# BurntSushi/aho-corasick

Measured on NVIDIA B200. Metric: haystack_scan_throughput, higher is better.
Workload: dtype u8

## Files before the change

### aho-corasick_b200/csrc/acb_api.cu

```cuda
#include <cuda_runtime.h>

#include <algorithm>
#include <chrono>
#include <cstdio>
#include <cstdlib>
#include <cstring>
#include <atomic>
#include <pthread.h>
#include <condition_variable>
#include <functional>
#include <mutex>
#include <thread>
#include <new>
#include <vector>

#include "../../include/acb200.h"
#include "../../include/acb200_debug.h"
#include "acb_build.hpp"
#include "acb_comm.hpp"
#include "acb_device.cuh"

using acb::DfaDev;
using acb::HostDfa;

namespace {

#define CK(expr)                                                                       \
  do {                                                                                 \
    cudaError_t e_ = (expr);                                                           \
    if (e_ != cudaSuccess) {                                                           \
      std::fprintf(stderr, "acb200: CUDA error %s at %s:%d: %s\n", cudaGetErrorName(e_), \
                   __FILE__, __LINE__, cudaGetErrorString(e_));                        \
      return ACG_E_CUDA;                                                               \
    }                                                                                  \
  } while (0)

struct Workspace {
  cudaStream_t stream = nullptr, copy_stream = nullptr;
  cudaEvent_t ev0 = nullptr, ev1 = nullptr, ev2 = nullptr, ev3 = nullptr;
  uint64_t cap = 0;
  uint64_t* d_keys[2] = {nullptr, nullptr};
  uint32_t* d_pids[2] = {nullptr, nullptr};
  unsigned long long* d_counter = nullptr;
  unsigned long long* h_counter = nullptr;
  void* d_temp = nullptr;
  size_t temp_bytes = 0;
  uint64_t* h_keys = nullptr;
  uint32_t* h_pids = nullptr;
  uint64_t h_cap = 0;
  uint8_t* d_hay = nullptr;
  uint64_t d_hay_cap = 0;
  uint64_t* d_scratch = nullptr;
  uint8_t* d_flags = nullptr;
  void* d_temp2 = nullptr;
  size_t temp2_bytes = 0;
  uint64_t chain_cap = 0;
  uint64_t* d_seq = nullptr;
  uint64_t seq_cap = 0;
  uint64_t* h_seq = nullptr;
  uint64_t h_seq_cap = 0;
  acg_stats stats{};
  uint8_t* h_stage[2] = {nullptr, nullptr};
  uint64_t h_stage_cap = 0;
  cudaEvent_t stage_ev[2] = {nullptr, nullptr};
};

}

struct PrefilterPlan {
  bool supported = false;
  uint32_t k = 0, kmask = 0, fold = 0, mult = 1, mult3 = 1, shift = 0, log_bits = 0;
  uint32_t stride = 1;
  uint32_t key_shift = 8;
  bool wide = false;
  bool brute = false;
  uint32_t dup_shift = 0;
  double fill = 0;
  uint64_t n_grams = 0;
  std::vector<uint32_t> bitmap;
  bool dense = false;
  std::vector<uint64_t> amap;
  uint32_t amap_log = 0;
  uint32_t bs_n = 0;
  uint8_t bs_byte[3] = {0, 0, 0};
  uint8_t bs_back[3] = {0, 0, 0};
};

struct acg_dfa {
  HostDfa h;
  std::vector<uint16_t> depth16;
  PrefilterPlan pf;
  uint32_t* d_bitmap = nullptr;
  uint2* d_amap = nullptr;
  bool has_empty = false;
  uint32_t max_list_len = 0;
  bool on_device = false;
  bool dev_touched = false;
  int device = -1;
  uint32_t* d_trans = nullptr;
  uint8_t* d_classes = nullptr;
  uint32_t* d_moff = nullptr;
  uint32_t* d_mpids = nullptr;
  uint32_t* d_plens = nullptr;
  uint16_t* d_depth16 = nullptr;
  DfaDev dev{};
  int engine_override = ACG_ENGINE_AUTO;
  uint64_t pipeline_chunk = 64ull << 20;
  mutable bool bytescan_inert = false;
  uint32_t experiment = 0;
  mutable std::mutex mu;
  static constexpr size_t kMaxWorkspaces = 4;
  mutable std::vector<Workspace*> ws_all, ws_free;
  mutable std::condition_variable ws_cv;
  mutable acg_stats last_stats{};
};

namespace {

thread_local Workspace* tls_ws = nullptr;
thread_local const acg_dfa* tls_stats_owner = nullptr;
thread_local acg_stats tls_stats{};
Workspace& cur_ws() { return *tls_ws; }

int init_workspace(Workspace& w) {
  CK(cudaStreamCreateWithFlags(&w.stream, cudaStreamNonBlocking));
  CK(cudaStreamCreateWithFlags(&w.copy_stream, cudaStreamNonBlocking));
  CK(cudaEventCreate(&w.ev0));
  CK(cudaEventCreate(&w.ev1));
  CK(cudaEventCreate(&w.ev2));
  CK(cudaEventCreate(&w.ev3));
  CK(cudaMalloc(&w.d_counter, 64));
  CK(cudaMallocHost(&w.h_counter, 64));
  return ACG_OK;
}

void destroy_workspace(Workspace& w) {
  if (w.stream) cudaStreamSynchronize(w.stream);
  for (int i = 0; i < 2; ++i) { cudaFree(w.d_keys[i]); cudaFree(w.d_pids[i]); }
  cudaFree(w.d_counter); cudaFree(w.d_temp); cudaFree(w.d_hay); cudaFree(w.d_seq);
  cudaFree(w.d_scratch); cudaFree(w.d_flags); cudaFree(w.d_temp2);
  if (w.h_counter) cudaFreeHost(w.h_counter);
  if (w.h_keys) cudaFreeHost(w.h_keys);
  if (w.h_pids) cudaFreeHost(w.h_pids);
  if (w.h_seq) cudaFreeHost(w.h_seq);
  for (int i = 0; i < 2; ++i) {
    if (w.h_stage[i]) cudaFreeHost(w.h_stage[i]);
    if (w.stage_ev[i]) cudaEventDestroy(w.stage_ev[i]);
  }
  if (w.ev0) cudaEventDestroy(w.ev0);
  if (w.ev1) cudaEventDestroy(w.ev1);
  if (w.ev2) cudaEventDestroy(w.ev2);
  if (w.ev3) cudaEventDestroy(w.ev3);
  if (w.stream) cudaStreamDestroy(w.stream);
  if (w.copy_stream) cudaStreamDestroy(w.copy_stream);
}

struct WsLease {
  const acg_dfa* a;
  Workspace* w = nullptr;
  Workspace* prev;
  int rc = ACG_OK;
  explicit WsLease(const acg_dfa* a_) : a(a_), prev(tls_ws) {
    std::unique_lock<std::mutex> lk(a->mu);
    for (;;) {
      if (!a->ws_free.empty()) { w = a->ws_free.back(); a->ws_free.pop_back(); break; }
      if (a->ws_all.size() < acg_dfa::kMaxWorkspaces) {
        w = new (std::nothrow) Workspace();
        if (!w) { rc = ACG_E_NOMEM; return; }
        a->ws_all.push_back(w);
        lk.unlock();
        int prev_dev = -1;
        cudaGetDevice(&prev_dev);
        if (prev_dev != a->device) cudaSetDevice(a->device);
        rc = init_workspace(*w);
        if (prev_dev != a->device && prev_dev >= 0) cudaSetDevice(prev_dev);
        break;
      }
      a->ws_cv.wait(lk);
    }
    if (rc == ACG_OK) { w->stats = acg_stats{}; tls_ws = w; }
  }
  Workspace* detach() {
    Workspace* out = w;
    if (w) { tls_stats = w->stats; tls_stats_owner = a; tls_ws = prev; }
    w = nullptr;
    return out;
  }
  ~WsLease() {
    if (!w) return;
    tls_stats = w->stats;
    tls_stats_owner = a;
    tls_ws = prev;
    std::lock_guard<std::mutex> lk(a->mu);
    a->last_stats = w->stats;
    if (rc == ACG_OK) a->ws_free.push_back(w);
    a->ws_cv.notify_one();
  }
};

void release_workspace(const acg_dfa* a, Workspace* w) {
  if (!w) return;
  std::lock_guard<std::mutex> lk(a->mu);
  a->last_stats = w->stats;
  a->ws_free.push_back(w);
  a->ws_cv.notify_one();
}

int bits_for(uint64_t v) {
  int b = 0;
  while (v) { ++b; v >>= 1; }
  return b;
}

uint32_t bloom_hash2(uint32_t x) {
  x ^= x >> 16;
  x *= 0x7feb352du;
  x ^= x >> 15;
  x *= 0x846ca68bu;
  x ^= x >> 16;
  return x;
}

// ... 412 lines not shown
}

int ensure_tuple_cap(Workspace& w, uint64_t cap) {
  if (cap <= w.cap) return ACG_OK;
  for (int i = 0; i < 2; ++i) {
    if (w.d_keys[i]) cudaFree(w.d_keys[i]);
    if (w.d_pids[i]) cudaFree(w.d_pids[i]);
    w.d_keys[i] = nullptr;
    w.d_pids[i] = nullptr;
  }
  if (w.d_temp) { cudaFree(w.d_temp); w.d_temp = nullptr; }
  w.cap = 0;
  for (int i = 0; i < 2; ++i) {
    CK(cudaMalloc(&w.d_keys[i], cap * 8));
    CK(cudaMalloc(&w.d_pids[i], cap * 4));
  }
  size_t tb = 0;
  CK(acb::sort_pairs(nullptr, tb, w.d_keys[0], w.d_keys[1], w.d_pids[0], w.d_pids[1], cap, 64, w.stream));
  CK(cudaMalloc(&w.d_temp, std::max<size_t>(tb, 16)));
  w.temp_bytes = tb;
  w.cap = cap;
  return ACG_OK;
}

int ensure_host_staging(Workspace& w, uint64_t n) {
  if (n <= w.h_cap) return ACG_OK;
  if (w.h_keys) cudaFreeHost(w.h_keys);
  if (w.h_pids) cudaFreeHost(w.h_pids);
  w.h_keys = nullptr;
  w.h_pids = nullptr;
  w.h_cap = 0;
  const uint64_t cap = std::max<uint64_t>(n, 1 << 16);
  CK(cudaMallocHost(&w.h_keys, cap * 8));
  CK(cudaMallocHost(&w.h_pids, cap * 4));
  w.h_cap = cap;
  return ACG_OK;
}

int ensure_hay(Workspace& w, uint64_t bytes) {
  if (bytes <= w.d_hay_cap) return ACG_OK;
  if (w.d_hay) cudaFree(w.d_hay);
  w.d_hay = nullptr;
  w.d_hay_cap = 0;
  const uint64_t cap = ((bytes + (1ull << 20)) >> 20) << 20;
  CK(cudaMalloc(&w.d_hay, cap));
  w.d_hay_cap = cap;
  return ACG_OK;
}

int ensure_seq(Workspace& w, uint64_t cap) {
  if (cap > w.seq_cap) {
    if (w.d_seq) cudaFree(w.d_seq);
    w.d_seq = nullptr;
    w.seq_cap = 0;
    CK(cudaMalloc(&w.d_seq, cap * 24));
    w.seq_cap = cap;
  }
  if (cap > w.h_seq_cap) {
    if (w.h_seq) cudaFreeHost(w.h_seq);
    w.h_seq = nullptr;
    w.h_seq_cap = 0;
    CK(cudaMallocHost(&w.h_seq, cap * 24));
    w.h_seq_cap = cap;
  }
  return ACG_OK;
}

int check_anchored(int have, int want_anchored) {
  if (have == ACG_START_BOTH) return ACG_OK;
  if (have == ACG_START_UNANCHORED) return want_anchored ? ACG_E_INVALID_INPUT_ANCHORED : ACG_OK;
  return want_anchored ? ACG_OK : ACG_E_INVALID_INPUT_UNANCHORED;
}
bool span_ok(uint64_t hay_len, uint64_t s, uint64_t e) { return e <= hay_len && s <= e + 1; }
int check_start(const HostDfa& h, int anchored) {
  if (anchored) return h.start_anchored_id == 0 ? ACG_E_INVALID_INPUT_ANCHORED : ACG_OK;
  return h.start_unanchored_id == 0 ? ACG_E_INVALID_INPUT_UNANCHORED : ACG_OK;
}

struct TupleResult {
  uint64_t n = 0;
  int sorted_buf = 0;
};

int run_walk_overlapping(const acg_dfa* a, const uint8_t* d_hay, uint64_t readable, uint64_t span_start,
                         uint64_t span_end, TupleResult* res) {
  Workspace& w = cur_ws();
  const uint64_t n_bytes = span_end - span_start;
  if (a->max_list_len >= (1u << acb::kTieBits)) return ACG_E_INVALID_ARG;
  if (n_bytes >= (1ull << (64 - acb::kTieBits))) return ACG_E_INVALID_ARG;
  int dev_sms = 148;
  cudaDeviceGetAttribute(&dev_sms, cudaDevAttrMultiProcessorCount, a->device);
  const uint64_t target_lanes = uint64_t(dev_sms) * 2048;
  uint64_t seg_len = (n_bytes + target_lanes - 1) / std::max<uint64_t>(target_lanes, 1);
  seg_len = std::max<uint64_t>(seg_len, 256);
  seg_len = (seg_len + 15) & ~15ull;
  const uint64_t n_segs = std::max<uint64_t>((n_bytes + seg_len - 1) / seg_len, 1);
  uint64_t cap = std::max<uint64_t>(w.cap, std::max<uint64_t>(1 << 20, n_bytes / 256));
  for (int attempt = 0; attempt < 8; ++attempt) {
    int rc = ensure_tuple_cap(w, cap);
    if (rc) return rc;
    CK(cudaMemsetAsync(w.d_counter, 0, 8, w.stream));
    acb::WalkLaunch p;
    p.hay = d_hay;
    p.hay_len = readable;
    p.span_start = span_start;
    p.span_end = span_end;
    p.seg_len = seg_len;
    p.n_segs = n_segs;
    p.keys = w.d_keys[0];
    p.pids = w.d_pids[0];
    p.counter = w.d_counter;
    p.cap = w.cap;
    CK(cudaEventRecord(w.ev0, w.stream));
    CK(acb::launch_walk_overlapping(a->dev, p, w.stream));
    CK(cudaEventRecord(w.ev1, w.stream));
    CK(cudaMemcpyAsync(w.h_counter, w.d_counter, 8, cudaMemcpyDeviceToHost, w.stream));
    CK(cudaStreamSynchronize(w.stream));
    cur_ws().stats.launches += 1;
    const uint64_t want = *w.h_counter;
    if (want > w.cap) { cap = want + want / 8 + 1024; continue; }
    res->n = want;
    cur_ws().stats.raw_matches = want;
    float ms = 0;
    cudaEventElapsedTime(&ms, w.ev0, w.ev1);
    cur_ws().stats.scan_ms = ms;
    if (want > 1) {
      size_t tb = w.temp_bytes;
      const int end_bit = std::min(64, acb::kTieBits + bits_for(n_bytes + 1));
      CK(cudaEventRecord(w.ev2, w.stream));
      CK(acb::sort_pairs(w.d_temp, tb, w.d_keys[0], w.d_keys[1], w.d_pids[0], w.d_pids[1], want, end_bit,
                         w.stream));
      CK(cudaEventRecord(w.ev3, w.stream));
      CK(cudaStreamSynchronize(w.stream));
      cudaEventElapsedTime(&ms, w.ev2, w.ev3);
      cur_ws().stats.order_ms = ms;
      cur_ws().stats.launches += 8;
      res->sorted_buf = 1;
    } else {
      res->sorted_buf = 0;
    }
    return ACG_OK;
  }
  return ACG_E_NOMEM;
}

int enqueue_prefilter_range(const acg_dfa* a, const uint8_t* d_hay, uint64_t readable,
                            uint64_t span_start, uint64_t span_end, uint64_t scan_lo,
                            uint64_t scan_hi, int mode, int dev_sms) {
  Workspace& w = cur_ws();
  const PrefilterPlan& pf = a->pf;
  const uintptr_t base = reinterpret_cast<uintptr_t>(d_hay);
  uint64_t lo = scan_lo + ((16 - ((base + scan_lo) & 15)) & 15);
  const uint64_t limit = std::min<uint64_t>(scan_hi, readable >= 20 ? readable - 20 : 0);
  uint64_t hi = lo;
  if (limit > lo) hi = lo + ((limit - lo) & ~15ull);
  if (lo > scan_hi) { lo = scan_hi; hi = scan_hi; }
  acb::PrefilterLaunch p;
  p.hay = d_hay;
  p.hay_len = readable;
  p.span_start = span_start;
  p.span_end = span_end;
  p.bitmap = a->d_bitmap;
  p.log_bits = pf.log_bits;
  p.k = pf.k;
  p.stride = pf.stride;
  p.geom = pf.wide ? 1 : 0;
  p.pair = 0;
  p.dyn = (a->experiment & ACG_EXP_STATIC_TILES) ? 0 : ((a->experiment & ACG_EXP_GLOBAL_TILES) ? 2 : 1);
  p.kmask = pf.kmask;
  p.fold = pf.fold;
  p.mult = pf.mult;
  p.mult3 = pf.mult3;
  p.key_shift = pf.key_shift;
  p.shift = pf.shift;
  p.dense = pf.dense ? 1 : 0;
  p.brute = pf.brute ? 1 : 0;
  p.mode = mode == 1 ? 1 : 0;
  p.first_only = mode == 2 ? 1 : 0;
  p.dup_shift = pf.dup_shift;
  p.scan_lo = scan_lo;
  p.scan_hi = scan_hi;
  p.region_lo = lo;
  p.region_hi = hi;
  p.keys = w.d_keys[0];
  p.pids = w.d_pids[0];
  p.counter = w.d_counter;
  p.cap = w.cap;
  p.bs_n = 0;
  for (int i = 0; i < 3; ++i) { p.bs_needle[i] = 0; p.bs_back[i] = 0; }
  if (pf.bs_n && !a->bytescan_inert && !(a->experiment & ACG_EXP_NO_BYTESCAN)) {
    p.bs_n = pf.bs_n;
    for (uint32_t i = 0; i < pf.bs_n; ++i) { p.bs_needle[i] = uint32_t(pf.bs_byte[i]) * 0x01010101u; p.bs_back[i] = pf.bs_back[i]; }
    CK(acb::launch_bytescan(a->dev, p, dev_sms, w.stream));
  } else {
    if (p.dyn == 2) CK(cudaMemsetAsync(w.d_counter + 2, 0, 8, w.stream));
    CK(acb::launch_prefilter(a->dev, p, dev_sms, w.stream));
  }
  cur_ws().stats.launches += 1;
  return ACG_OK;
}

int order_tuples(const acg_dfa* a, uint64_t want, uint64_t n_bytes, TupleResult* res) {
  Workspace& w = cur_ws();
  res->n = want;
  cur_ws().stats.raw_matches = want;
  if (want > 1) {
    size_t tb = w.temp_bytes;
    const int end_bit = std::min(64, acb::kTieBits + bits_for(n_bytes + 1));
    float ms = 0;
    CK(cudaEventRecord(w.ev2, w.stream));
    CK(acb::sort_pairs(w.d_temp, tb, w.d_keys[0], w.d_keys[1], w.d_pids[0], w.d_pids[1], want, end_bit,
                       w.stream));
    CK(cudaEventRecord(w.ev3, w.stream));
    CK(cudaStreamSynchronize(w.stream));
    cudaEventElapsedTime(&ms, w.ev2, w.ev3);
    cur_ws().stats.order_ms = ms;
    cur_ws().stats.launches += 8;
    res->sorted_buf = 1;
  } else {
    res->sorted_buf = 0;
  }
  return ACG_OK;
}

class CopyPool {
 public:
  static CopyPool& get() {
    static std::once_flag once;
    std::call_once(once, [] { pthread_atfork(nullptr, nullptr, [] { instance().store(nullptr); }); });
    CopyPool* p = instance().load(std::memory_order_acquire);
    if (!p) {
      CopyPool* fresh = new CopyPool;
      if (instance().compare_exchange_strong(p, fresh)) p = fresh;
    }
    return *p;
  }
  void copy(uint8_t* dst, const uint8_t* src, size_t n) {
    if (n < (4u << 20) || workers_.empty()) { std::memcpy(dst, src, n); return; }
    std::unique_lock<std::mutex> lk(mu_);
    busy_cv_.wait(lk, [&] { return !active_; });
    active_ = true;
    dst_ = dst; src_ = src; n_ = n;
    next_.store(0);
    pending_ = int(workers_.size());
    ++epoch_;
    cv_.notify_all();
    done_cv_.wait(lk, [&] { return pending_ == 0; });
    active_ = false;
    busy_cv_.notify_one();
  }

 private:
  static std::atomic<CopyPool*>& instance() {
    static std::atomic<CopyPool*> p{nullptr};
    return p;
  }
  CopyPool() {
    unsigned n = std::thread::hardware_concurrency();
    n = n >= 16 ? 8 : (n >= 4 ? n / 2 : 0);
    for (unsigned i = 0; i < n; ++i) workers_.emplace_back([this] { run(); });
    for (auto& t : workers_) t.detach();
  }
  void run() {
    uint64_t seen = 0;
    for (;;) {
      std::unique_lock<std::mutex> lk(mu_);
      cv_.wait(lk, [&] { return epoch_ != seen; });
      seen = epoch_;
      uint8_t* dst = dst_;
      const uint8_t* src = src_;
      const size_t n = n_;
      lk.unlock();
      constexpr size_t kSlice = 1u << 20;
      for (;;) {
        const size_t off = next_.fetch_add(kSlice);
        if (off >= n) break;
        std::memcpy(dst + off, src + off, std::min(kSlice, n - off));
      }
      lk.lock();
      if (--pending_ == 0) done_cv_.notify_one();
    }
  }
  std::mutex mu_;
  std::condition_variable cv_, done_cv_, busy_cv_;
  std::vector<std::thread> workers_;
  uint8_t* dst_ = nullptr;
  const uint8_t* src_ = nullptr;
  size_t n_ = 0;
  std::atomic<size_t> next_{0};
  int pending_ = 0;
  uint64_t epoch_ = 0;
  bool active_ = false;
};

bool is_pageable_host(const void* p) {
  cudaPointerAttributes attr;
  if (cudaPointerGetAttributes(&attr, p) != cudaSuccess) { cudaGetLastError(); return false; }
  return attr.type == cudaMemoryTypeUnregistered;
}

int ensure_stage(Workspace& w, uint64_t bytes) {
  if (bytes <= w.h_stage_cap) return ACG_OK;
  for (int i = 0; i < 2; ++i) {
    if (w.h_stage[i]) { cudaFreeHost(w.h_stage[i]); w.h_stage[i] = nullptr; }
    CK(cudaMallocHost(&w.h_stage[i], bytes));
    if (!w.stage_ev[i]) CK(cudaEventCreateWithFlags(&w.stage_ev[i], cudaEventDisableTiming));
  }
  w.h_stage_cap = bytes;
  return ACG_OK;
}

int run_prefilter(const acg_dfa* a, const uint8_t* d_hay, uint64_t readable, uint64_t span_start,
                  uint64_t span_end, int mode, TupleResult* res, const uint8_t* h_hay = nullptr,
                  uint64_t scan_lo = UINT64_MAX, uint64_t scan_hi = UINT64_MAX) {
  if (scan_lo == UINT64_MAX) { scan_lo = span_start; scan_hi = span_end; }
  Workspace& w = cur_ws();
  const uint64_t n_bytes = span_end - span_start;
  if (n_bytes >= (1ull << (64 - acb::kTieBits))) return ACG_E_INVALID_ARG;
  int dev_sms = 148;
  cudaDeviceGetAttribute(&dev_sms, cudaDevAttrMultiProcessorCount, a->device);
  uint64_t cap = std::max<uint64_t>(w.cap, std::max<uint64_t>(1 << 20, (scan_hi - scan_lo) / 256));
  bool copied = h_hay == nullptr;
  for (int attempt = 0; attempt < 8; ++attempt) {
    int rc = ensure_tuple_cap(w, cap);
    if (rc) return rc;
    CK(cudaMemsetAsync(w.d_counter, 0, 16, w.stream));
    CK(cudaEventRecord(w.ev0, w.stream));
    if (copied) {
      if ((rc = enqueue_prefilter_range(a, d_hay, readable, span_start, span_end, scan_lo, scan_hi, mode,
                                        dev_sms)))
        return rc;
    } else {
      const uint64_t chunk = a->pipeline_chunk;
      const uint64_t tail = std::min<uint64_t>(a->h.max_pattern_len, 1u << 30) + 64;
      uint64_t scanned = span_start;
      const bool staged = span_end - span_start >= std::min<uint64_t>(8u << 20, chunk) && is_pageable_host(h_hay + span_start);
      if (staged && (rc = ensure_stage(w, std::min<uint64_t>(chunk, span_end - span_start)))) return rc;
      bool stage_used[2] = {false, false};
      int stage_i = 0;
      CK(cudaEventRecord(w.ev2, w.copy_stream));
      for (uint64_t c0 = span_start; c0 < span_end; c0 += chunk) {
        const uint64_t c1 = std::min(span_end, c0 + chunk);
        const uint8_t* src = h_hay + c0;
        if (staged) {
          if (stage_used[stage_i]) CK(cudaEventSynchronize(w.stage_ev[stage_i]));
          CopyPool::get().copy(w.h_stage[stage_i], h_hay + c0, size_t(c1 - c0));
          src = w.h_stage[stage_i];
        }
        CK(cudaMemcpyAsync(const_cast<uint8_t*>(d_hay) + c0, src, c1 - c0, cudaMemcpyHostToDevice,
                           w.copy_stream));
        if (staged) {
          CK(cudaEventRecord(w.stage_ev[stage_i], w.copy_stream));
          stage_used[stage_i] = true;
          stage_i ^= 1;
        }
        CK(cudaEventRecord(w.ev3, w.copy_stream));
        CK(cudaStreamWaitEvent(w.stream, w.ev3, 0));
        const uint64_t upto = c1 == span_end ? span_end : (c1 > scanned + tail ? c1 - tail : scanned);
        if (upto > scanned || c1 == span_end) {
          if ((rc = enqueue_prefilter_range(a, d_hay, c1 == span_end ? readable : c1, span_start, span_end,
                                            scanned, upto, mode, dev_sms)))
            return rc;
          scanned = upto;
        }
      }
      copied = true;
    }
    CK(cudaEventRecord(w.ev1, w.stream));
    CK(cudaMemcpyAsync(w.h_counter, w.d_counter, 16, cudaMemcpyDeviceToHost, w.stream));
    CK(cudaStreamSynchronize(w.stream));
    const uint64_t want = w.h_counter[0];
    cur_ws().stats.candidates = w.h_counter[1];
    if (a->pf.bs_n && !a->bytescan_inert && scan_hi - scan_lo >= (1u << 16) && w.h_counter[1] > (scan_hi - scan_lo) / 64)
      a->bytescan_inert = true;
    float ms = 0;
    cudaEventElapsedTime(&ms, w.ev0, w.ev1);
    cur_ws().stats.scan_ms = ms;
    if (want > w.cap) { cap = want + want / 8 + 1024; continue; }
    return order_tuples(a, want, n_bytes, res);
  }
  return ACG_E_NOMEM;
}

int ensure_chain(Workspace& w, uint64_t n) {
  if (n <= w.chain_cap) return ACG_OK;
  if (w.d_scratch) cudaFree(w.d_scratch);
  if (w.d_flags) cudaFree(w.d_flags);
  if (w.d_temp2) cudaFree(w.d_temp2);
  w.d_scratch = nullptr; w.d_flags = nullptr; w.d_temp2 = nullptr; w.chain_cap = 0;
  const uint64_t cap = std::max<uint64_t>(n, 1 << 16);
  CK(cudaMalloc(&w.d_scratch, cap * 8));
  CK(cudaMalloc(&w.d_flags, cap));
  size_t t1 = 0, t2 = 0;
  CK(acb::scan_max_u64(nullptr, t1, w.d_scratch, cap, w.stream));
  CK(acb::select_flagged(nullptr, t2, w.d_keys[0], w.d_pids[0], w.d_flags, w.d_keys[1], w.d_pids[1],
                         w.d_counter, cap, w.stream));
  w.temp2_bytes = std::max(t1, t2);
  CK(cudaMalloc(&w.d_temp2, std::max<size_t>(w.temp2_bytes, 16)));
  w.chain_cap = cap;
  return ACG_OK;
}

int run_chain(const acg_dfa* a, int mode, TupleResult* r) {
  Workspace& w = cur_ws();
  if (r->n == 0) return ACG_OK;
  int rc = ensure_chain(w, r->n);
  if (rc) return rc;
  const int src = r->sorted_buf, dst = 1 - src;
  acb::ChainLaunch c;
  c.keys = w.d_keys[src];
  c.pids = w.d_pids[src];
  c.pattern_lens = a->d_plens;
  c.n = r->n;
  c.mode = mode;
  c.scratch_end = w.d_scratch;
  c.flags = w.d_flags;
  CK(cudaEventRecord(w.ev2, w.stream));
  CK(cudaMemsetAsync(w.d_flags, 0, r->n, w.stream));
  CK(acb::launch_chain_ends(c, w.stream));
  size_t tb = w.temp2_bytes;
  CK(acb::scan_max_u64(w.d_temp2, tb, w.d_scratch, r->n, w.stream));
  CK(acb::launch_chain_select(c, w.stream));
  tb = w.temp2_bytes;
  CK(acb::select_flagged(w.d_temp2, tb, w.d_keys[src], w.d_pids[src], w.d_flags, w.d_keys[dst],
                         w.d_pids[dst], w.d_counter, r->n, w.stream));
  CK(cudaEventRecord(w.ev3, w.stream));
  CK(cudaMemcpyAsync(w.h_counter, w.d_counter, 8, cudaMemcpyDeviceToHost, w.stream));
  CK(cudaStreamSynchronize(w.stream));
  float ms = 0;
  cudaEventElapsedTime(&ms, w.ev2, w.ev3);
  cur_ws().stats.order_ms += ms;
  cur_ws().stats.launches += 8;
  r->n = *w.h_counter;
  r->sorted_buf = dst;
  return ACG_OK;
}

int drain_tuples(const acg_dfa* a, const TupleResult& r, uint64_t span_start, acg_match* out,
                 uint64_t cap, uint64_t* n_out, uint64_t* fnv, int key_mode = 0) {
  Workspace& w = cur_ws();
  *n_out = r.n;
  if (fnv) *fnv = 0xcbf29ce484222325ull;
  if (r.n == 0) return ACG_OK;
  if (!fnv && r.n > cap) return ACG_E_OVERFLOW;
  int rc = ensure_host_staging(w, r.n);
  if (rc) return rc;
  CK(cudaEventRecord(w.ev0, w.stream));
  CK(cudaMemcpyAsync(w.h_keys, w.d_keys[r.sorted_buf], r.n * 8, cudaMemcpyDeviceToHost, w.stream));
  CK(cudaMemcpyAsync(w.h_pids, w.d_pids[r.sorted_buf], r.n * 4, cudaMemcpyDeviceToHost, w.stream));
  CK(cudaEventRecord(w.ev1, w.stream));
  CK(cudaStreamSynchronize(w.stream));
  float ms = 0;
  cudaEventElapsedTime(&ms, w.ev0, w.ev1);
  cur_ws().stats.d2h_ms += ms;
  const uint32_t* plens = a->h.pattern_lens.data();
  uint64_t hsh = 0xcbf29ce484222325ull;
  auto mix = [&](uint64_t v) {
    for (int k = 0; k < 8; ++k) { hsh ^= (v >> (8 * k)) & 0xFF; hsh *= 0x100000001b3ull; }
  };
  for (uint64_t i = 0; i < r.n; ++i) {
    const uint32_t pid = w.h_pids[i];
    uint64_t start, end;
// ... 541 lines not shown
  if (cudaMemcpy(t.data(), a->d_trans, t.size() * 4, cudaMemcpyDeviceToHost) != cudaSuccess) {
    cudaGetLastError();
    return ACG_E_CUDA;
  }
  h.trans.swap(t);
  return ACG_OK;
}

}

int acg_dfa_table(const acg_dfa* a, acg_dfa_desc* o) {
  if (!a || !o) return ACG_E_INVALID_ARG;
  if (int rc = fetch_table(a)) return rc;
  const HostDfa& h = a->h;
  o->trans = h.trans.data();
  o->trans_len = h.trans.size();
  o->stride2 = h.stride2;
  o->alphabet_len = h.alphabet_len;
  std::memcpy(o->byte_classes, h.classes, 256);
  o->max_special_id = h.max_special_id;
  o->max_match_id = h.max_match_id;
  o->start_unanchored_id = h.start_unanchored_id;
  o->start_anchored_id = h.start_anchored_id;
  o->match_offsets = h.match_offsets.data();
  o->match_pids = h.match_pids.data();
  o->pattern_lens = h.pattern_lens.data();
  o->n_patterns = uint32_t(h.pattern_lens.size());
  o->match_kind = uint32_t(h.match_kind);
  o->start_kind = uint32_t(h.start_kind);
  o->prefilter_kind = uint32_t(h.prefilter_kind);
  o->min_pattern_len = h.min_pattern_len;
  o->max_pattern_len = h.max_pattern_len;
  return ACG_OK;
}

uint64_t acg_dfa_state_len(const acg_dfa* a) { return a ? a->h.state_len : 0; }
int acg_kind(const acg_dfa* a) { return a ? a->h.reported_kind : 0; }
int acg_match_kind(const acg_dfa* a) { return a ? a->h.match_kind : 0; }
int acg_start_kind(const acg_dfa* a) { return a ? a->h.start_kind : 0; }
uint64_t acg_patterns_len(const acg_dfa* a) { return a ? a->h.pattern_lens.size() : 0; }
uint64_t acg_min_pattern_len(const acg_dfa* a) { return a ? a->h.min_pattern_len : 0; }
uint64_t acg_max_pattern_len(const acg_dfa* a) { return a ? a->h.max_pattern_len : 0; }
uint64_t acg_memory_usage(const acg_dfa* a) {
  if (!a) return 0;
  const HostDfa& h = a->h;
  return h.trans_len * 4 + (h.match_offsets.size() - 1) * 24 + h.match_pids.size() * 4 +
         h.pattern_lens.size() * 4;
}
int acg_prefilter_kind(const acg_dfa* a) { return a ? a->h.prefilter_kind : 0; }
int acg_packed_variant(const acg_dfa* a, int* fat, int* mask_len) {
  if (!a || !a->h.packed.active) return 0;
  if (fat) *fat = a->h.packed.fat;
  if (mask_len) *mask_len = a->h.packed.mask_len;
  return 1;
}

int acg_debug_prefilter_plan(const acg_dfa* a, acg_prefilter_plan* out) {
  if (!a || !out) return ACG_E_INVALID_ARG;
  const PrefilterPlan& pf = a->pf;
  *out = acg_prefilter_plan{};
  out->supported = pf.supported ? 1 : 0;
  out->brute = pf.brute ? 1 : 0;
  out->dense = pf.dense ? 1 : 0;
  out->stride = int32_t(pf.stride);
  out->wide = pf.wide ? 1 : 0;
  out->k = pf.k; out->kmask = pf.kmask; out->fold = pf.fold;
  out->mult = pf.mult; out->mult3 = pf.mult3; out->key_shift = pf.key_shift; out->shift = pf.shift; out->log_bits = pf.log_bits;
  out->bitmap = pf.bitmap.data(); out->bitmap_words = pf.bitmap.size();
  out->amap = pf.amap.data(); out->amap_log = pf.amap_log;
  out->depth16 = a->depth16.data(); out->n_rows = a->depth16.size();
  out->dup_shift = pf.dup_shift;
  out->bs_n = (pf.bs_n && !a->bytescan_inert) ? pf.bs_n : 0;
  for (int i = 0; i < 3; ++i) { out->bs_byte[i] = pf.bs_byte[i]; out->bs_back[i] = pf.bs_back[i]; }
  return ACG_OK;
}

int acg_debug_set_pipeline_chunk(acg_dfa* a, uint64_t bytes) {
  if (!a || bytes < 4096 || (bytes & 4095)) return ACG_E_INVALID_ARG;
  a->pipeline_chunk = bytes;
  return ACG_OK;
}

int acg_debug_set_experiment(acg_dfa* a, uint32_t flags) {
  if (!a || (flags & ~uint32_t(ACG_EXP_KEY24 | ACG_EXP_STATIC_TILES | ACG_EXP_NO_BYTESCAN | ACG_EXP_GLOBAL_TILES))) return ACG_E_INVALID_ARG;
  std::lock_guard<std::mutex> lock(a->mu);
  const uint32_t changed = a->experiment ^ flags;
  a->experiment = flags;
  if (changed & ACG_EXP_KEY24) {
    const size_t old_words = a->pf.bitmap.size();
    derive_metadata(a);
    if (a->on_device && a->d_bitmap && a->pf.supported) {
      if (a->pf.bitmap.size() != old_words) return ACG_E_INVALID_ARG;
      DeviceGuard guard(a->device);
      if (cudaMemcpy(a->d_bitmap, a->pf.bitmap.data(), old_words * 4, cudaMemcpyHostToDevice) != cudaSuccess) {
        cudaGetLastError();
        return ACG_E_CUDA;
      }
    }
  }
  return ACG_OK;
}

int acg_set_engine(acg_dfa* a, int engine) {
  if (!a || engine < ACG_ENGINE_AUTO || engine > ACG_ENGINE_SEQUENTIAL) return ACG_E_INVALID_ARG;
  a->engine_override = engine;
  return ACG_OK;
}
static acg_stats stats_for(const acg_dfa* a) {
  if (tls_stats_owner == a) return tls_stats;
  std::lock_guard<std::mutex> lk(a->mu);
  return a->last_stats;
}
int acg_last_engine(const acg_dfa* a) { return a ? stats_for(a).engine : 0; }
int acg_last_stats(const acg_dfa* a, acg_stats* out) {
  if (!a || !out) return ACG_E_INVALID_ARG;
  *out = stats_for(a);
  return ACG_OK;
}

int acg_find_overlapping(const acg_dfa* a, const uint8_t* hay, uint64_t hay_len, uint64_t span_start,
                         uint64_t span_end, int anchored, acg_match* out, uint64_t cap,
                         uint64_t* n_out) {
  return overlapping_impl(a, hay, false, hay_len, span_start, span_end, anchored, out, cap, n_out,
                          nullptr, nullptr);
}
int acg_find_overlapping_dev(const acg_dfa* a, const void* d_hay, uint64_t hay_len,
                             uint64_t span_start, uint64_t span_end, acg_match* out, uint64_t cap,
                             uint64_t* n_out, float* kernel_ms) {
  return overlapping_impl(a, static_cast<const uint8_t*>(d_hay), true, hay_len, span_start, span_end,
                          0, out, cap, n_out, nullptr, kernel_ms);
}
int acg_find_overlapping_devout(const acg_dfa* a, const void* d_hay, uint64_t hay_len,
                                uint64_t span_start, uint64_t span_end, uint64_t min_end,
                                uint64_t offset_add, void* d_out, uint64_t cap, uint64_t* n_out,
                                float* kernel_ms) {
  if (!d_out && cap) return ACG_E_INVALID_ARG;
  DevOut dv;
  dv.d_out = d_out;
  dv.min_end = min_end;
  dv.offset_add = offset_add;
  return overlapping_impl(a, static_cast<const uint8_t*>(d_hay), true, hay_len, span_start, span_end, 0,
                          nullptr, cap, n_out, nullptr, kernel_ms, &dv);
}
int acg_count_overlapping_dev(const acg_dfa* a, const void* d_hay, uint64_t hay_len,
                              uint64_t span_start, uint64_t span_end, uint64_t* n_out, uint64_t* fnv,
                              float* kernel_ms) {
  uint64_t dummy_fnv = 0;
  return overlapping_impl(a, static_cast<const uint8_t*>(d_hay), true, hay_len, span_start, span_end,
                          0, nullptr, 0, n_out, fnv ? fnv : &dummy_fnv, kernel_ms);
}

int acg_find_iter(const acg_dfa* a, const uint8_t* hay, uint64_t hay_len, uint64_t span_start,
                  uint64_t span_end, int anchored, acg_match* out, uint64_t cap, uint64_t* n_out) {
  return find_iter_impl(a, hay, false, hay_len, span_start, span_end, anchored, out, cap, n_out,
                        nullptr);
}
int acg_find_iter_dev(const acg_dfa* a, const void* d_hay, uint64_t hay_len, uint64_t span_start,
                      uint64_t span_end, acg_match* out, uint64_t cap, uint64_t* n_out,
                      float* kernel_ms) {
  return find_iter_impl(a, static_cast<const uint8_t*>(d_hay), true, hay_len, span_start, span_end, 0,
                        out, cap, n_out, kernel_ms);
}

int acg_find(const acg_dfa* a, const uint8_t* hay, uint64_t hay_len, uint64_t span_start,
             uint64_t span_end, int anchored, int earliest, acg_match* out, int* found) {
  if (!out || !found) return ACG_E_INVALID_ARG;
  *found = 0;
// ... 349 lines not shown
```

### aho-corasick_b200/csrc/acb_device.cuh

```cuda
#pragma once
#include <cuda_runtime.h>
#include <stdint.h>

namespace acb {

constexpr int kTieBits = 24;
constexpr uint64_t kTieMask = (1ull << kTieBits) - 1;
constexpr uint64_t kInvalidKey = ~0ull;

struct DfaDev {
  const uint32_t* trans;
  const uint8_t* classes;
  const uint32_t* match_offsets;
  const uint32_t* match_pids;
  const uint32_t* pattern_lens;
  const uint16_t* depth16;
  uint32_t stride2;
  uint32_t max_match_id;
  uint32_t start_unanchored_id;
  uint32_t start_anchored_id;
  uint32_t max_pattern_len;
  uint32_t min_pattern_len;
  const uint2* amap;
  uint32_t amap_shift;
// ... 28 lines not shown
  uint32_t n;
};
cudaError_t launch_dfa_fill_level(const FillLaunch& f, cudaStream_t s);

struct SeqLaunch {
  const uint8_t* hay;
  uint64_t span_start, span_end;
  int anchored;
  int match_kind;
  int earliest;
  int single;
  uint64_t* out;
  unsigned long long* counter;
  uint64_t cap;
};
cudaError_t launch_seq_find(const DfaDev& dfa, const SeqLaunch& p, cudaStream_t s);

struct PrefilterLaunch {
  const uint8_t* hay;
  uint64_t hay_len;
  uint64_t span_start, span_end;
  const uint32_t* bitmap;
  uint32_t log_bits;
  uint32_t k;
  uint32_t stride;
  uint16_t geom;
  uint16_t pair;
  uint32_t kmask;
  uint32_t fold;
  uint32_t mult;
  uint32_t mult3;
  uint32_t shift;
  int dense;
  int brute;
  int mode;
  int first_only;
  uint32_t dup_shift;
  uint64_t scan_lo, scan_hi;
  uint64_t region_lo, region_hi;
  uint64_t* keys;
  uint32_t* pids;
  unsigned long long* counter;
  uint64_t cap;
  uint32_t dyn;
  uint32_t bs_n;
  uint32_t bs_needle[3];
  uint32_t bs_back[3];
  uint32_t key_shift;
};
cudaError_t launch_prefilter(const DfaDev& dfa, const PrefilterLaunch& p, int sm_count, cudaStream_t s);
cudaError_t launch_bytescan(const DfaDev& dfa, const PrefilterLaunch& p, int sm_count, cudaStream_t s);

struct ChainLaunch {
  const uint64_t* keys;
  const uint32_t* pids;
  const uint32_t* pattern_lens;
  uint64_t n;
  int mode;
  uint64_t* scratch_end;
  uint8_t* flags;
};
cudaError_t launch_chain_ends(const ChainLaunch& c, cudaStream_t s);
cudaError_t launch_chain_select(const ChainLaunch& c, cudaStream_t s);
cudaError_t scan_max_u64(void* d_temp, size_t& temp_bytes, uint64_t* data, uint64_t n, cudaStream_t s);
cudaError_t select_flagged(void* d_temp, size_t& temp_bytes, const uint64_t* keys_in, const uint32_t* pids_in,
                           const uint8_t* flags, uint64_t* keys_out, uint32_t* pids_out,
                           unsigned long long* d_num_out, uint64_t n, cudaStream_t s);

struct ExpandLaunch {
  const uint64_t* keys;
  const uint32_t* pids;
  const uint32_t* pattern_lens;
  uint64_t n;
  uint64_t first;
  uint64_t span_start;
  uint64_t offset_add;
  uint64_t* out;
  int small = 0;
};
cudaError_t launch_expand(const ExpandLaunch& e, cudaStream_t s);
cudaError_t launch_lower_bound(const uint64_t* keys, uint64_t n, uint64_t bound_key,
                               unsigned long long* d_result, cudaStream_t s);

cudaError_t sort_pairs(void* d_temp, size_t& temp_bytes, const uint64_t* keys_in, uint64_t* keys_out,
                       const uint32_t* vals_in, uint32_t* vals_out, uint64_t n, int end_bit,
                       cudaStream_t s);

}
```

### aho-corasick_b200/csrc/acb_kernels.cu

```cuda
#include "acb_device.cuh"
#ifndef ACB_PTX_HEADER
#define ACB_PTX_HEADER "acb_ptx.cuh"
#endif
#include ACB_PTX_HEADER

#include <algorithm>
#include <cstdio>
#include <cstdlib>

#include <cub/device/device_radix_sort.cuh>

namespace acb {

namespace {

__device__ __noinline__ void emit_state_matches(const uint32_t* match_offsets, const uint32_t* match_pids,
                                                uint32_t row, uint64_t end_rel, uint64_t* keys, uint32_t* pids,
                                                unsigned long long* counter, uint64_t cap) {
  const uint32_t lo = match_offsets[row], hi = match_offsets[row + 1];
  const int lane = threadIdx.x & 31;
  for (uint32_t i = lo; i < hi; ++i) {
    const unsigned m = __activemask();
    const int leader = __ffs(m) - 1;
    unsigned long long base = 0;
// ... 120 lines not shown
    sid = d.trans[sid + d.classes[hay[at]]];
    if (sid <= d.max_match_id) {
      if (sid == 0) break;
      SeqMatch m = seq_get_match(d, sid, 0, at + 1);
      if (!(anchored && m.start > start)) {
        mat = m;
        have = true;
        if (earliest) break;
      }
    }
    ++at;
  }
  if (have) *out = mat;
  return have;
}

__global__ void seq_find_kernel(DfaDev d, SeqLaunch p) {
  if (threadIdx.x != 0 || blockIdx.x != 0) return;
  const bool anchored = p.anchored != 0;
  const bool earliest = p.match_kind == 0 || p.earliest != 0;
  uint64_t start = p.span_start;
  unsigned long long n = 0;
  bool have_last = false;
  uint64_t last_end = 0;
  for (;;) {
    SeqMatch m;
    if (!seq_try_find(d, p.hay, start, p.span_end, anchored, earliest, &m)) break;
    if (!p.single && m.start == m.end && have_last && m.end == last_end) {
      start += 1;
      if (!seq_try_find(d, p.hay, start, p.span_end, anchored, earliest, &m)) break;
    }
    if (n < p.cap) {
      p.out[n * 3 + 0] = m.pid;
      p.out[n * 3 + 1] = m.start;
      p.out[n * 3 + 2] = m.end;
    }
    ++n;
    if (p.single) break;
    start = m.end;
    last_end = m.end;
    have_last = true;
  }
  *p.counter = n;
}

template <int kExpandThreads>
__global__ void __launch_bounds__(kExpandThreads) expand_kernel(ExpandLaunch e) {
  __shared__ uint64_t s_rec[kExpandThreads * 3];
  const uint64_t m = e.n - e.first;
  for (uint64_t base = (uint64_t)blockIdx.x * kExpandThreads; base < m; base += (uint64_t)gridDim.x * kExpandThreads) {
    const uint64_t i = base + threadIdx.x;
    if (i < m) {
      const uint64_t key = e.keys[e.first + i];
      const uint32_t pid = e.pids[e.first + i];
      const uint64_t end = e.span_start + (key >> kTieBits) + e.offset_add;
      s_rec[threadIdx.x * 3 + 0] = (uint64_t)pid;
      s_rec[threadIdx.x * 3 + 1] = end - e.pattern_lens[pid];
      s_rec[threadIdx.x * 3 + 2] = end;
    }
    __syncthreads();
    const uint64_t cnt = m - base < kExpandThreads ? m - base : kExpandThreads;
    uint64_t* dst = e.out + base * 3;
    const uint32_t words = (uint32_t)cnt * 3;
    const uint32_t head = (uint32_t)((reinterpret_cast<uintptr_t>(dst) >> 3) & 1);
    if (head && threadIdx.x == 0 && words) dst[0] = s_rec[0];
    for (uint32_t w = head + threadIdx.x * 2; w + 1 < words; w += 2 * kExpandThreads)
      *reinterpret_cast<ulonglong2*>(dst + w) = make_ulonglong2(s_rec[w], s_rec[w + 1]);
    if (words > head && ((words - head) & 1) && threadIdx.x == 0) dst[words - 1] = s_rec[words - 1];
    __syncthreads();
  }
}

__global__ void lower_bound_kernel(const uint64_t* keys, uint64_t n, uint64_t bound_key,
                                   unsigned long long* result) {
  if (threadIdx.x != 0 || blockIdx.x != 0) return;
  uint64_t lo = 0, hi = n;
  while (lo < hi) {
    const uint64_t mid = lo + (hi - lo) / 2;
    if (keys[mid] < bound_key) lo = mid + 1; else hi = mid;
  }
  *result = lo;
}

}

cudaError_t launch_expand(const ExpandLaunch& e, cudaStream_t s) {
  const uint64_t m = e.n - e.first;
  if (m == 0) return cudaSuccess;
  if (e.small) {
    const uint64_t blocks = (m + 127) / 128;
    ACB_LAUNCH(expand_kernel<128>, (unsigned)(blocks < (uint64_t)e.small ? blocks : (uint64_t)e.small), 128, 0, s, e);
  } else {
    ACB_LAUNCH(expand_kernel<256>, (unsigned)((m + 255) / 256), 256, 0, s, e);
  }
  return cudaGetLastError();
}
cudaError_t launch_lower_bound(const uint64_t* keys, uint64_t n, uint64_t bound_key,
                               unsigned long long* d_result, cudaStream_t s) {
  ACB_LAUNCH(lower_bound_kernel, 1, 32, 0, s, keys, n, bound_key, d_result);
  return cudaGetLastError();
}

cudaError_t launch_walk_overlapping(const DfaDev& dfa, const WalkLaunch& p, cudaStream_t s) {
  const uint64_t blocks = (p.n_segs + kWalkThreads - 1) / kWalkThreads;
  ACB_LAUNCH(walk_overlapping_kernel, (unsigned)blocks, kWalkThreads, 0, s, dfa, p);
  return cudaGetLastError();
}

cudaError_t launch_dfa_fill_level(const FillLaunch& f, cudaStream_t s) {
  if (f.n == 0) return cudaSuccess;
#ifdef ACB_EMULATE
  if (getenv("ACB_EMU_TRACE")) fprintf(stderr, "launch_dfa_fill_level rows %u\n", f.n);
#endif
  const uint64_t blocks = ((uint64_t)f.n * 32 + kFillThreads - 1) / kFillThreads;
  ACB_LAUNCH(dfa_fill_level_kernel, (unsigned)blocks, kFillThreads, 0, s, f);
  return cudaGetLastError();
}


cudaError_t launch_seq_find(const DfaDev& dfa, const SeqLaunch& p, cudaStream_t s) {
  ACB_LAUNCH(seq_find_kernel, 1, 32, 0, s, dfa, p);
  return cudaGetLastError();
}

cudaError_t sort_pairs(void* d_temp, size_t& temp_bytes, const uint64_t* keys_in, uint64_t* keys_out,
                       const uint32_t* vals_in, uint32_t* vals_out, uint64_t n, int end_bit,
                       cudaStream_t s) {
  return cub::DeviceRadixSort::SortPairs(d_temp, temp_bytes, keys_in, keys_out, vals_in, vals_out, n,
                                         0, end_bit, s);
}

}
```

### include/acb200_debug.h

```cpp
#ifndef ACB200_DEBUG_H
#define ACB200_DEBUG_H

#include "acb200.h"

#ifdef __cplusplus
extern "C" {
#endif

typedef struct {
  int32_t supported;
  int32_t brute;
  int32_t dense;
  int32_t stride;
  int32_t wide;
  uint32_t k;
  uint32_t kmask, fold, mult, mult3, shift, log_bits;
  const uint32_t* bitmap;
  uint64_t bitmap_words;
  const uint64_t* amap;
  uint32_t amap_log;
  const uint16_t* depth16;
  uint64_t n_rows;
  uint32_t dup_shift;
  uint32_t key_shift;
  uint32_t bs_n;
  uint8_t bs_byte[3];
  uint8_t bs_back[3];
} acg_prefilter_plan;

int acg_debug_prefilter_plan(const acg_dfa* dfa, acg_prefilter_plan* out);

int acg_debug_set_pipeline_chunk(acg_dfa* dfa, uint64_t bytes);

#define ACG_EXP_KEY24 8u
#define ACG_EXP_STATIC_TILES 32u
#define ACG_EXP_GLOBAL_TILES 16u
#define ACG_EXP_NO_BYTESCAN 64u
int acg_debug_set_experiment(acg_dfa* dfa, uint32_t flags);

#ifdef __cplusplus
}
#endif
#endif
```

Baseline: 1987.

## Replace CUB radix sort of match tuples with bucketed counting sort

Match tuples are now ordered by a custom pipeline instead of a full CUB radix sort over all key bits. The pipeline histograms keys into coarse offset buckets, scans the counts, scatters tuples into their buckets, then sorts each bucket in shared memory with a sub-bucket count plus rank pass. It also narrows the tie bits from the pattern-list length so fewer key bits are involved. If a bucket overflows, too many buckets are needed, or a new experiment flag is set, it falls back to CUB, which costs an extra host sync and a wasted pass.

```diff
diff --git a/aho-corasick_b200/csrc/acb_api.cu b/aho-corasick_b200/csrc/acb_api.cu
--- a/aho-corasick_b200/csrc/acb_api.cu
+++ b/aho-corasick_b200/csrc/acb_api.cu
@@ -45,6 +45,7 @@
   unsigned long long* h_counter = nullptr;
   void* d_temp = nullptr;
   size_t temp_bytes = 0;
+  uint32_t* d_order = nullptr;
   uint64_t* h_keys = nullptr;
   uint32_t* h_pids = nullptr;
   uint64_t h_cap = 0;
@@ -131,13 +132,14 @@
   CK(cudaEventCreate(&w.ev3));
   CK(cudaMalloc(&w.d_counter, 64));
   CK(cudaMallocHost(&w.h_counter, 64));
+  CK(cudaMalloc(&w.d_order, 2 * (size_t(acb::kOrderMaxBuckets) + 1) * 4));
   return ACG_OK;
 }
 
 void destroy_workspace(Workspace& w) {
   if (w.stream) cudaStreamSynchronize(w.stream);
   for (int i = 0; i < 2; ++i) { cudaFree(w.d_keys[i]); cudaFree(w.d_pids[i]); }
-  cudaFree(w.d_counter); cudaFree(w.d_temp); cudaFree(w.d_hay); cudaFree(w.d_seq);
+  cudaFree(w.d_counter); cudaFree(w.d_temp); cudaFree(w.d_order); cudaFree(w.d_hay); cudaFree(w.d_seq);
   cudaFree(w.d_scratch); cudaFree(w.d_flags); cudaFree(w.d_temp2);
   if (w.h_counter) cudaFreeHost(w.h_counter);
   if (w.h_keys) cudaFreeHost(w.h_keys);
@@ -716,6 +718,54 @@
   int sorted_buf = 0;
 };
 
+int order_tuples(const acg_dfa* a, uint64_t want, uint64_t n_bytes, int tie_bits, TupleResult* res) {
+  Workspace& w = cur_ws();
+  res->n = want;
+  w.stats.raw_matches = want;
+  res->sorted_buf = 0;
+  if (want <= 1) return ACG_OK;
+  const int offset_bits = bits_for(n_bytes + 1);
+  int off_bits = std::min(offset_bits, 32 - tie_bits);
+  while (off_bits > 0 && ((n_bytes >> off_bits) + 1) * acb::kOrderBucketTarget < want) --off_bits;
+  const uint64_t n_buckets = (n_bytes >> off_bits) + 1;
+  bool fallback = (a->experiment & ACG_EXP_CUB_ORDER) || n_buckets > acb::kOrderMaxBuckets;
+  CK(cudaEventRecord(w.ev2, w.stream));
+  if (!fallback) {
+    acb::OrderLaunch o;
+    o.keys_in = w.d_keys[0];
+    o.pids_in = w.d_pids[0];
+    o.keys_out = w.d_keys[1];
+    o.pids_out = w.d_pids[1];
+    o.n = want;
+    o.bucket_shift = uint32_t(acb::kTieBits + off_bits);
+    o.n_buckets = uint32_t(n_buckets);
+    o.tie_bits = uint32_t(tie_bits);
+    o.counts = w.d_order;
+    o.starts = w.d_order + acb::kOrderMaxBuckets + 1;
+    o.overflow = w.d_counter + 3;
+    CK(acb::launch_order(o, w.stream));
+    CK(cudaEventRecord(w.ev3, w.stream));
+    CK(cudaMemcpyAsync(w.h_counter + 3, w.d_counter + 3, 8, cudaMemcpyDeviceToHost, w.stream));
+    CK(cudaStreamSynchronize(w.stream));
+    w.stats.launches += 4;
+    fallback = w.h_counter[3] != 0;
+  }
+  if (fallback) {
+    size_t tb = w.temp_bytes;
+    const int end_bit = std::min(64, acb::kTieBits + offset_bits);
+    CK(acb::sort_pairs(w.d_temp, tb, w.d_keys[0], w.d_keys[1], w.d_pids[0], w.d_pids[1], want, end_bit,
+                       w.stream));
+    CK(cudaEventRecord(w.ev3, w.stream));
+    CK(cudaStreamSynchronize(w.stream));
+    w.stats.launches += 2 + (end_bit + 7) / 8;
+  }
+  float ms = 0;
+  cudaEventElapsedTime(&ms, w.ev2, w.ev3);
+  w.stats.order_ms = ms;
+  res->sorted_buf = 1;
+  return ACG_OK;
+}
+
 int run_walk_overlapping(const acg_dfa* a, const uint8_t* d_hay, uint64_t readable, uint64_t span_start,
                          uint64_t span_end, TupleResult* res) {
   Workspace& w = cur_ws();
@@ -753,27 +803,10 @@
     cur_ws().stats.launches += 1;
     const uint64_t want = *w.h_counter;
     if (want > w.cap) { cap = want + want / 8 + 1024; continue; }
-    res->n = want;
-    cur_ws().stats.raw_matches = want;
     float ms = 0;
     cudaEventElapsedTime(&ms, w.ev0, w.ev1);
     cur_ws().stats.scan_ms = ms;
-    if (want > 1) {
-      size_t tb = w.temp_bytes;
-      const int end_bit = std::min(64, acb::kTieBits + bits_for(n_bytes + 1));
-      CK(cudaEventRecord(w.ev2, w.stream));
-      CK(acb::sort_pairs(w.d_temp, tb, w.d_keys[0], w.d_keys[1], w.d_pids[0], w.d_pids[1], want, end_bit,
-                         w.stream));
-      CK(cudaEventRecord(w.ev3, w.stream));
-      CK(cudaStreamSynchronize(w.stream));
-      cudaEventElapsedTime(&ms, w.ev2, w.ev3);
-      cur_ws().stats.order_ms = ms;
-      cur_ws().stats.launches += 8;
-      res->sorted_buf = 1;
-    } else {
-      res->sorted_buf = 0;
-    }
-    return ACG_OK;
+    return order_tuples(a, want, n_bytes, bits_for(a->max_list_len), res);
   }
   return ACG_E_NOMEM;
 }
@@ -831,29 +864,6 @@
     CK(acb::launch_prefilter(a->dev, p, dev_sms, w.stream));
   }
   cur_ws().stats.launches += 1;
-  return ACG_OK;
-}
-
-int order_tuples(const acg_dfa* a, uint64_t want, uint64_t n_bytes, TupleResult* res) {
-  Workspace& w = cur_ws();
-  res->n = want;
-  cur_ws().stats.raw_matches = want;
-  if (want > 1) {
-    size_t tb = w.temp_bytes;
-    const int end_bit = std::min(64, acb::kTieBits + bits_for(n_bytes + 1));
-    float ms = 0;
-    CK(cudaEventRecord(w.ev2, w.stream));
-    CK(acb::sort_pairs(w.d_temp, tb, w.d_keys[0], w.d_keys[1], w.d_pids[0], w.d_pids[1], want, end_bit,
-                       w.stream));
-    CK(cudaEventRecord(w.ev3, w.stream));
-    CK(cudaStreamSynchronize(w.stream));
-    cudaEventElapsedTime(&ms, w.ev2, w.ev3);
-    cur_ws().stats.order_ms = ms;
-    cur_ws().stats.launches += 8;
-    res->sorted_buf = 1;
-  } else {
-    res->sorted_buf = 0;
-  }
   return ACG_OK;
 }
 
@@ -1011,7 +1021,7 @@
     cudaEventElapsedTime(&ms, w.ev0, w.ev1);
     cur_ws().stats.scan_ms = ms;
     if (want > w.cap) { cap = want + want / 8 + 1024; continue; }
-    return order_tuples(a, want, n_bytes, res);
+    return order_tuples(a, want, n_bytes, bits_for(a->h.max_pattern_len) + int(a->pf.dup_shift), res);
   }
   return ACG_E_NOMEM;
 }
@@ -1719,7 +1729,9 @@
 }
 
 int acg_debug_set_experiment(acg_dfa* a, uint32_t flags) {
-  if (!a || (flags & ~uint32_t(ACG_EXP_KEY24 | ACG_EXP_STATIC_TILES | ACG_EXP_NO_BYTESCAN | ACG_EXP_GLOBAL_TILES))) return ACG_E_INVALID_ARG;
+  if (!a || (flags & ~uint32_t(ACG_EXP_KEY24 | ACG_EXP_STATIC_TILES | ACG_EXP_NO_BYTESCAN | ACG_EXP_GLOBAL_TILES |
+                               ACG_EXP_CUB_ORDER)))
+    return ACG_E_INVALID_ARG;
   std::lock_guard<std::mutex> lock(a->mu);
   const uint32_t changed = a->experiment ^ flags;
   a->experiment = flags;
diff --git a/aho-corasick_b200/csrc/acb_device.cuh b/aho-corasick_b200/csrc/acb_device.cuh
--- a/aho-corasick_b200/csrc/acb_device.cuh
+++ b/aho-corasick_b200/csrc/acb_device.cuh
@@ -134,6 +134,23 @@
 cudaError_t launch_lower_bound(const uint64_t* keys, uint64_t n, uint64_t bound_key,
                                unsigned long long* d_result, cudaStream_t s);
 
+constexpr uint32_t kOrderMaxBuckets = 8192;
+constexpr uint64_t kOrderBucketTarget = 2048;
+struct OrderLaunch {
+  const uint64_t* keys_in;
+  const uint32_t* pids_in;
+  uint64_t* keys_out;
+  uint32_t* pids_out;
+  uint64_t n;
+  uint32_t bucket_shift;
+  uint32_t n_buckets;
+  uint32_t tie_bits;
+  uint32_t* counts;
+  uint32_t* starts;
+  unsigned long long* overflow;
+};
+cudaError_t launch_order(const OrderLaunch& o, cudaStream_t s);
+
 cudaError_t sort_pairs(void* d_temp, size_t& temp_bytes, const uint64_t* keys_in, uint64_t* keys_out,
                        const uint32_t* vals_in, uint32_t* vals_out, uint64_t n, int end_bit,
                        cudaStream_t s);
diff --git a/aho-corasick_b200/csrc/acb_kernels.cu b/aho-corasick_b200/csrc/acb_kernels.cu
--- a/aho-corasick_b200/csrc/acb_kernels.cu
+++ b/aho-corasick_b200/csrc/acb_kernels.cu
@@ -226,6 +226,169 @@
   *result = lo;
 }
 
+constexpr int kBucketThreads = 512;
+constexpr int kBucketItems = 16;
+constexpr int kScanThreads = 1024;
+constexpr int kSortThreads = 256;
+constexpr int kSortItems = 16;
+constexpr uint32_t kSortCapacity = kSortThreads * kSortItems;
+constexpr uint32_t kSubBucketLimit = 1024;
+
+__device__ __forceinline__ uint32_t bucket_of(const OrderLaunch& o, uint64_t key) {
+  const uint64_t b = key >> o.bucket_shift;
+  return (b < o.n_buckets && ((key & kTieMask) >> o.tie_bits) == 0) ? (uint32_t)b : o.n_buckets;
+}
+
+__device__ __forceinline__ uint32_t block_exclusive_sum(uint32_t v, uint32_t* s_warp) {
+  const uint32_t lane = threadIdx.x & 31, warp = threadIdx.x >> 5;
+  uint32_t x = v;
+  for (uint32_t d = 1; d < 32; d <<= 1) {
+    const uint32_t y = (uint32_t)__shfl_sync(0xffffffffu, x, (lane - d) & 31);
+    if (lane >= d) x += y;
+  }
+  if (lane == 31) s_warp[warp] = x;
+  __syncthreads();
+  for (uint32_t w = 0; w < warp; ++w) x += s_warp[w];
+  __syncthreads();
+  return x - v;
+}
+
+template <bool kScatter>
+__global__ void __launch_bounds__(kBucketThreads) order_bucket_kernel(OrderLaunch o) {
+  ACB_DYNAMIC_SMEM(smem);
+  uint32_t* hist = reinterpret_cast<uint32_t*>(smem);
+  if (kScatter && *o.overflow) return;
+  for (uint32_t b = threadIdx.x; b <= o.n_buckets; b += kBucketThreads) hist[b] = 0;
+  __syncthreads();
+  const uint64_t base = (uint64_t)blockIdx.x * (kBucketThreads * kBucketItems) + threadIdx.x;
+  uint64_t key[kBucketItems];
+  uint32_t pid[kBucketItems], rank[kBucketItems];
+#pragma unroll
+  for (int j = 0; j < kBucketItems; ++j) {
+    const uint64_t i = base + (uint64_t)j * kBucketThreads;
+    if (i < o.n) {
+      key[j] = o.keys_in[i];
+      if (kScatter) pid[j] = o.pids_in[i];
+    }
+  }
+#pragma unroll
+  for (int j = 0; j < kBucketItems; ++j)
+    if (base + (uint64_t)j * kBucketThreads < o.n) rank[j] = atomicAdd(&hist[bucket_of(o, key[j])], 1u);
+  __syncthreads();
+  for (uint32_t b = threadIdx.x; b <= o.n_buckets; b += kBucketThreads) {
+    const uint32_t c = hist[b];
+    if (c) {
+      const uint32_t at = atomicAdd(&o.counts[b], c);
+      if (kScatter) hist[b] = at;
+    }
+  }
+  if (!kScatter) return;
+  __syncthreads();
+#pragma unroll
+  for (int j = 0; j < kBucketItems; ++j) {
+    const uint64_t i = base + (uint64_t)j * kBucketThreads;
+    if (i < o.n) {
+      const uint32_t at = hist[bucket_of(o, key[j])] + rank[j];
+      o.keys_out[at] = key[j];
+      o.pids_out[at] = pid[j];
+    }
+  }
+}
+
+__global__ void __launch_bounds__(kScanThreads) order_scan_kernel(OrderLaunch o, uint32_t capacity) {
+  __shared__ uint32_t s_warp[kScanThreads / 32];
+  __shared__ uint32_t s_bad;
+  if (threadIdx.x == 0) s_bad = o.counts[o.n_buckets] != 0;
+  const uint32_t per = (o.n_buckets + kScanThreads - 1) / kScanThreads;
+  const uint32_t lo = threadIdx.x * per < o.n_buckets ? threadIdx.x * per : o.n_buckets;
+  const uint32_t hi = lo + per < o.n_buckets ? lo + per : o.n_buckets;
+  uint32_t sum = 0;
+  bool bad = false;
+  for (uint32_t b = lo; b < hi; ++b) {
+    const uint32_t c = o.counts[b];
+    sum += c;
+    bad |= c > capacity;
+  }
+  __syncthreads();
+  if (bad) s_bad = 1;
+  uint32_t run = block_exclusive_sum(sum, s_warp);
+  for (uint32_t b = lo; b < hi; ++b) {
+    const uint32_t c = o.counts[b];
+    o.starts[b] = run;
+    o.counts[b] = run;
+    run += c;
+  }
+  if (threadIdx.x == kScanThreads - 1) o.starts[o.n_buckets] = run;
+  if (threadIdx.x == 0) *o.overflow = s_bad;
+}
+
+__global__ void __launch_bounds__(kSortThreads, 4) order_sort_kernel(OrderLaunch o, uint32_t capacity) {
+  __shared__ uint32_t s_start[kSortThreads + 1];
+  __shared__ uint32_t s_warp[kSortThreads / 32];
+  __shared__ uint32_t s_big;
+  if (*o.overflow) return;
+  const uint32_t bucket = blockIdx.x;
+  const uint32_t first = o.starts[bucket], n = o.starts[bucket + 1] - first;
+  if (n <= 1) return;
+  ACB_DYNAMIC_SMEM(smem);
+  uint32_t* sk = reinterpret_cast<uint32_t*>(smem);
+  uint32_t* sp = sk + capacity;
+  const uint32_t off_bits = o.bucket_shift - kTieBits, tie_bits = o.tie_bits;
+  const uint32_t dshift = off_bits + tie_bits > 8 ? off_bits + tie_bits - 8 : 0;
+  const uint64_t off_mask = (1ull << off_bits) - 1, tie_mask = (1ull << tie_bits) - 1;
+  uint64_t* keys = o.keys_out + first;
+  uint32_t* pids = o.pids_out + first;
+  s_start[threadIdx.x] = 0;
+  if (threadIdx.x == 0) s_big = 0;
+  __syncthreads();
+  uint64_t key[kSortItems];
+  uint32_t local[kSortItems], pid[kSortItems], rank[kSortItems];
+#pragma unroll
+  for (int j = 0; j < kSortItems; ++j) {
+    const uint32_t i = j * kSortThreads + threadIdx.x;
+    if (i < n) {
+      key[j] = keys[i];
+      pid[j] = pids[i];
+    }
+  }
+#pragma unroll
+  for (int j = 0; j < kSortItems; ++j) {
+    if (j * kSortThreads + threadIdx.x < n) {
+      local[j] = (uint32_t)((((key[j] >> kTieBits) & off_mask) << tie_bits) | (key[j] & tie_mask));
+      rank[j] = atomicAdd(&s_start[local[j] >> dshift], 1u);
+    }
+  }
+  __syncthreads();
+  const uint32_t c = s_start[threadIdx.x];
+  if (c > kSubBucketLimit) s_big = 1;
+  const uint32_t at = block_exclusive_sum(c, s_warp);
+  if (s_big) {
+    if (threadIdx.x == 0) *o.overflow = 1;
+    return;
+  }
+  s_start[threadIdx.x] = at;
+  if (threadIdx.x == kSortThreads - 1) s_start[kSortThreads] = at + c;
+  __syncthreads();
+#pragma unroll
+  for (int j = 0; j < kSortItems; ++j) {
+    const uint32_t i = j * kSortThreads + threadIdx.x;
+    if (i < n) {
+      const uint32_t q = s_start[local[j] >> dshift] + rank[j];
+      sk[q] = local[j];
+      sp[q] = pid[j];
+    }
+  }
+  __syncthreads();
+  const uint64_t hi = (uint64_t)bucket << o.bucket_shift;
+  for (uint32_t q = threadIdx.x; q < n; q += kSortThreads) {
+    const uint32_t k = sk[q], d = k >> dshift;
+    uint32_t r = s_start[d];
+    for (uint32_t x = s_start[d], e = s_start[d + 1]; x < e; ++x) r += sk[x] < k || (sk[x] == k && x < q);
+    keys[r] = hi | ((uint64_t)(k >> tie_bits) << kTieBits) | (k & tie_mask);
+    pids[r] = sp[q];
+  }
+}
+
 }
 
 cudaError_t launch_expand(const ExpandLaunch& e, cudaStream_t s) {
@@ -267,6 +430,22 @@
   return cudaGetLastError();
 }
 
+cudaError_t launch_order(const OrderLaunch& o, cudaStream_t s) {
+  uint32_t capacity = kSortCapacity;
+#ifdef ACB_EMULATE
+  if (const char* e = getenv("ACB_EMU_ORDER_CAP")) capacity = (uint32_t)atoi(e);
+#endif
+  const size_t hist_smem = ((size_t)o.n_buckets + 1) * 4;
+  const uint64_t tiles = (o.n + kBucketThreads * kBucketItems - 1) / (kBucketThreads * kBucketItems);
+  cudaError_t e = cudaMemsetAsync(o.counts, 0, hist_smem, s);
+  if (e != cudaSuccess) return e;
+  ACB_LAUNCH(order_bucket_kernel<false>, (unsigned)tiles, kBucketThreads, hist_smem, s, o);
+  ACB_LAUNCH(order_scan_kernel, 1, kScanThreads, 0, s, o, capacity);
+  ACB_LAUNCH(order_bucket_kernel<true>, (unsigned)tiles, kBucketThreads, hist_smem, s, o);
+  ACB_LAUNCH(order_sort_kernel, o.n_buckets, kSortThreads, (size_t)capacity * 8, s, o, capacity);
+  return cudaGetLastError();
+}
+
 cudaError_t sort_pairs(void* d_temp, size_t& temp_bytes, const uint64_t* keys_in, uint64_t* keys_out,
                        const uint32_t* vals_in, uint32_t* vals_out, uint64_t n, int end_bit,
                        cudaStream_t s) {
diff --git a/include/acb200_debug.h b/include/acb200_debug.h
--- a/include/acb200_debug.h
+++ b/include/acb200_debug.h
@@ -36,6 +36,7 @@
 #define ACG_EXP_STATIC_TILES 32u
 #define ACG_EXP_GLOBAL_TILES 16u
 #define ACG_EXP_NO_BYTESCAN 64u
+#define ACG_EXP_CUB_ORDER 128u
 int acg_debug_set_experiment(acg_dfa* dfa, uint32_t flags);
 
 #ifdef __cplusplus
```

Result: faster. 2136 (median of 6 runs) (+7.5%).
